# mjq11302010044/TPGSR

Measured on AMD Instinct MI355X. Metric: training img/s (16x64->32x128, bs=48/GPU), TPGSR-TSRN full train step, higher is better.
Workload: dtype bf16x2; 1 GPU; C3: TPGSR-TSRN = TSRN_TL (STN+mask) + CRNN teacher/student text prior, stu_iter 1, full train step (teacher fwd, student fwd+bwd, distill loss, prior dropout, SR fwd+bwd, ImageLoss(gradient), clip 0.25, Adam); tpg=crnn, batch_per_gpu=48, global_batch=48, parallelism=dp1, launch=recorded plans, plain launches: main + weight-gradient + teacher streams

## Files before the change

### tpgsr_amd/csrc/conv_route.cpp

```cpp
#include "conv_route.h"
#include <stdint.h>
#include <stdlib.h>
#include <initializer_list>

static inline int cdiv(long long a, long long b) { return (int)((a + b - 1) / b); }

static bool env_off(const char* name) { const char* e = getenv(name); return e && e[0] == '0'; }
static bool env_on(const char* name) { const char* e = getenv(name); return e && e[0] == '1'; }
static long long env_ll(const char* name, long long dflt) { const char* e = getenv(name); return e ? atoll(e) : dflt; }

static ConvKnobs knobs_from_env() {
  ConvKnobs k;
  k.wstat = !env_off("TPGSR_CONV_WSTAT");
  const long long target = env_ll("TPGSR_WGRAD_TARGET", 0);
  k.wgrad_target = target > 0 ? target : 1024;
  k.halo3 = !env_off("TPGSR_XBF_HALO3");
  k.halo3_min_supertiles = env_ll("TPGSR_XBF_HALO3_MIN", 192);
  k.halo = !env_off("TPGSR_XBF_HALO");
  k.halo_min_taps = env_on("TPGSR_XBF_HALO_MINTAPS") ? 1 : 2;
  k.colmajor_min_bytes = 3ll << 20;
  k.panel = !env_off("TPGSR_XBF_PANEL");
  k.panel_min_m = env_ll("TPGSR_XBF_PANEL_MIN_M", 32768);
  k.panel_k192 = env_on("TPGSR_XBF_PANEL_K192");
  k.splitk = !env_off("TPGSR_XBF_SPLITK");
  k.splitk_target = (int)env_ll("TPGSR_XBF_SPLITK_TARGET", 640);
  k.splitk_min_chunks = (int)env_ll("TPGSR_XBF_SPLITK_MIN_CHUNKS", 6);
  k.splitk_max_tiles = (int)env_ll("TPGSR_XBF_SPLITK_MAX_TILES", 256);
  k.splitk_min_k = (int)env_ll("TPGSR_XBF_SPLITK_MIN_K", 24);
  k.splitk_over_halo = !env_off("TPGSR_XBF_SPLITK_OVER_HALO");
  k.wgrad3 = !env_off("TPGSR_XBF_WGRAD3");
  k.wgrad_halo = !env_off("TPGSR_XBF_WGRAD_HALO");
  k.wgrad_halo_minwork = env_ll("TPGSR_XBF_WGRAD_HALO_MINWORK", 16384);
  return k;
}
ConvKnobs g_conv_knobs = knobs_from_env();

extern "C" void tpgsr_halo3_set_enabled(int on) { g_conv_knobs.halo3 = on ? 1 : 0; }
extern "C" void tpgsr_halo_set_min_taps(int v) { g_conv_knobs.halo_min_taps = v < 1 ? 1 : v; }
extern "C" void tpgsr_halo_set_colmajor_min_bytes(long long v) { g_conv_knobs.colmajor_min_bytes = v; }
extern "C" void tpgsr_panel_set_enabled(int on) { g_conv_knobs.panel = on ? 1 : 0; }
extern "C" void tpgsr_panel_set_min_m(long long m) { g_conv_knobs.panel_min_m = m < 64 ? 64 : m; }
extern "C" void tpgsr_panel_set_k192(int on) { g_conv_knobs.panel_k192 = on ? 1 : 0; }
extern "C" void tpgsr_splitk_set_enabled(int on) { g_conv_knobs.splitk = on ? 1 : 0; }
extern "C" void tpgsr_wgrad3_set_enabled(int on) { g_conv_knobs.wgrad3 = on ? 1 : 0; }

int loader_bits(const tpgsr_conv_args* a) {
  return (a->in_scale ? 1 : 0) | (a->in_act ? 2 : 0) | (a->in2 ? 4 : 0) | (a->in_ps ? 8 : 0) | (a->in_b ? 16 : 0) | (a->in2_scale ? 32 : 0);
}

bool xbf_eligible(const tpgsr_conv_args* a) { return a->terms > 0 && a->wt_bf && (a->Cin & 3) == 0 && (a->wt_coff & 31) == 0; }

static int halo_capacity_of(const tpgsr_conv_args* a, int P) {
  const int Wp = a->OW + a->KW - 1, ohw = a->OH * a->OW;
  const int row_wraps = (a->OW % P == 0) ? 0 : (P - 1) / a->OW + 1;
  const int img_wraps = (ohw % P == 0) ? 0 : (P - 1) / ohw + 1;
  return P - 1 + row_wraps * (a->KW - 1) + img_wraps * (a->KH - 1) * Wp + (a->KH - 1) * Wp + a->KW;
}
int halo_capacity(const tpgsr_conv_args* a) { return halo_capacity_of(a, 64); }
int halo3_capacity(const tpgsr_conv_args* a) { return halo_capacity_of(a, 64 * kH3Tiles); }

void wgrad_plan(long long M, int K, int Cout, int* Z, int* MB) {
  const int kb = cdiv(K, kWgradWK), nb = cdiv(Cout, kConvBN);
  long long z = (g_conv_knobs.wgrad_target + (long long)kb * nb - 1) / ((long long)kb * nb);
  long long maxz = (M + 255) / 256;
  if (maxz > 256) maxz = 256;
  if (z > maxz) z = maxz;
  if (z < 1) z = 1;
  long long mb = (M + z - 1) / z;
  mb = (mb + kWgradWM - 1) / kWgradWM * kWgradWM;
  z = (M + mb - 1) / mb;
  *Z = (int)z;
  *MB = (int)mb;
}

int splitk_choice(long long M, int Cout, int kp) {
  const ConvKnobs& k = g_conv_knobs;
  const long long ntiles = cdiv(M, 64) * cdiv(Cout, 64);
  const int nchunks = kp / kConvKC;
  if (ntiles > k.splitk_max_tiles || nchunks < k.splitk_min_k) return 0;
  int S = (int)(k.splitk_target / ntiles);
  S = S < 2 ? 2 : S > 8 ? 8 : S;
  int cps = (nchunks + S - 1) / S;
  if (cps < k.splitk_min_chunks) cps = k.splitk_min_chunks;
  S = (nchunks + cps - 1) / cps;
  return S > 1 ? S : 0;
}

static constexpr unsigned long long ld_set(std::initializer_list<int> lds) {
  unsigned long long m = 0;
  for (int b : lds) m |= 1ull << b;
  return m;
}
static bool ld_in(int ld, unsigned long long set) { return (unsigned)ld < 64 && ((set >> ld) & 1); }
static constexpr unsigned long long kF32FwdLd = ld_set({0, 1, 2, 3, 4, 5, 7, 8, 17});
static constexpr unsigned long long kWgradTileLd = ld_set({0, 1, 2, 3, 4, 5, 7, 17});
static constexpr unsigned long long kXbfFwdLd = ld_set({0, 1, 2, 3, 4, 5, 7, 8, 17});
static constexpr unsigned long long kHaloLd = ld_set({0, 1, 2, 3, 4, 5, 7});
static constexpr unsigned long long kHalo3Ld = ld_set({0, 1, 2, 3, 4, 5, 7, 37});
static constexpr unsigned long long kPanelLd = ld_set({0, 1, 4, 17});
static constexpr unsigned long long kWgradBatchLd = ld_set({0, 1, 3});
bool wgrad_batch_has_ld(int ld) { return ld_in(ld, kWgradBatchLd); }

static int halo3_takes(const tpgsr_conv_args* a, long long M, int ld, int* lds_out) {
  const ConvKnobs& k = g_conv_knobs;
  const int T = a->terms, taps = a->KH * a->KW;
  if (!k.halo3 || T < 1 || T > 2 || taps < 3 || !(taps & 1) || a->wt_bf_cin != a->Cin || (a->Cin & 31) || a->stride_w > 1 || a->in_dil_w > 1 ||
      a->in_b || a->in_ps || !ld_in(ld, kHalo3Ld) || a->OW + a->KW - 1 < 8)
    return 0;
  if ((ld & 4) && a->out_ps) return 0;
  const int Lcap = halo3_capacity(a);
  const int lds = 2 * T * (32 * kH3Entries * 64) + 2 * kH3Tiles * 1024 + 8 * 4096;
  if (Lcap > 32 * kH3Entries || lds > 163840) return 0;
  const long long nst = (long long)cdiv(cdiv(M, 64), kH3Tiles) * cdiv(a->Cout, 64);
  if (nst < k.halo3_min_supertiles) return 0;
  *lds_out = lds;
  return Lcap;
}

static int halo_takes(const tpgsr_conv_args* a, int ld, int* lds_out) {
  const ConvKnobs& k = g_conv_knobs;
  const int taps = a->KH * a->KW;
  if (!k.halo || taps < k.halo_min_taps || (a->wt_bf_cin != a->Cin && !(taps == 1 && a->wt_bf_cin == 0)) || (a->Cin & 31) || a->stride_w > 1 ||
      a->in_dil_w > 1 || a->in_b || !(ld_in(ld, kHaloLd) || ld == 8) || a->OW + a->KW - 1 < 8)
    return 0;
  const int Lcap = halo_capacity(a);
  const long long lds = 2ll * a->terms * Lcap * 64 + 2048;
  if (Lcap > 32 * 7 || lds > 80 * 1024) return 0;
  *lds_out = (int)lds;
  return Lcap;
}

static int panel_takes(const tpgsr_conv_args* a, long long M, int ld, int* lds_out) {
  const ConvKnobs& k = g_conv_knobs;
  const int T = a->terms;
  if (!k.panel || a->KH * a->KW != 1 || a->wt_bf_cin != 0 || a->stride_w > 1 || a->in_dil_w > 1 || a->in_ps || a->pad_h || a->pad_w ||
      a->OH != a->H || a->OW != a->W || M < k.panel_min_m || T < 1 || T > 3)
    return 0;
  const int nb32 = (a->Cout + 31) >> 5, nq8 = a->kp >> 5;
  int nbw = 0;
  if ((nq8 == 2 || nq8 == 3) && nb32 <= 6) nbw = 3;
  else if (nq8 == 6 && nb32 <= 2 && k.panel_k192) nbw = 1;
  else return 0;
  if (!ld_in(ld, kPanelLd)) return 0;
  const int panel = T * 64 * (nq8 * 64 + 16), epilogue = (4 * 64 * nbw + 4 * 1024) * 4;
  *lds_out = panel > epilogue ? panel : epilogue;
  return nbw;
}

static bool wstat_takes(const tpgsr_conv_args* a, int ld) {
  return g_conv_knobs.wstat && ld == 0 && a->KH == 3 && a->KW == 3 && a->pad_h == 1 && a->pad_w == 1 && a->Cin == 64 && a->Cout == 64 &&
         a->W == 64 && a->OW == 64 && a->OH == a->H && a->in_dil_w <= 1 && a->stride_w <= 1 && !a->out_ps && a->out_act == TPGSR_ACT_NONE &&
         (a->wt_ld == 0 || a->wt_ld == 64) && a->wt_coff == 0 && (a->in_ld & 3) == 0 && (a->in_coff & 3) == 0 &&
         (((uintptr_t)a->in | (uintptr_t)a->wt) & 15) == 0;
}

static tpgsr_conv_route_t fwd_route(const tpgsr_conv_args* a, long long M, int ld, bool planning) {
  tpgsr_conv_route_t r = {};
  r.ld = ld;
  if (!xbf_eligible(a)) {
    const int wld = a->wt_ld > 0 ? a->wt_ld : a->Cout;
    const bool vecB = (wld & 3) == 0 && ((uintptr_t)a->wt & 15) == 0 && (a->wt_coff & 3) == 0;
    if (wstat_takes(a, ld)) {
      r.kernel = TPGSR_CONV_F32_WSTAT;
      r.lds_bytes = kWstatLdsBytes;
    } else if ((a->Cin & 3) != 0 || !vecB) {
      r.kernel = TPGSR_CONV_F32_SCALAR;
    } else {
      r.kernel = ld_in(ld, kF32FwdLd) ? TPGSR_CONV_F32_TILE : TPGSR_CONV_NONE;
    }
    return r;
  }
  if (!planning && a->sk_splits > 1) {
    r.kernel = ld_in(ld, kXbfFwdLd) ? TPGSR_CONV_XBF_SPLITK : TPGSR_CONV_NONE;
    r.splits = r.kernel ? a->sk_splits : 0;
    return r;
  }
  if ((r.lcap = halo3_takes(a, M, ld, &r.lds_bytes)) > 0) r.kernel = TPGSR_CONV_XBF_HALO3;
  else if ((r.lcap = halo_takes(a, ld, &r.lds_bytes)) > 0) r.kernel = TPGSR_CONV_XBF_HALO;
  else if ((r.nbw = panel_takes(a, M, ld, &r.lds_bytes)) > 0) r.kernel = TPGSR_CONV_XBF_PANEL;
  else r.kernel = ld_in(ld, kXbfFwdLd) ? TPGSR_CONV_XBF_TILE : TPGSR_CONV_NONE;
  int unused = 0;
  const ConvKnobs& k = g_conv_knobs;
  if (planning && k.splitk && a->terms <= 3 && a->bn_row_tiles <= 1 && !a->in2_scale && ld_in(ld, kXbfFwdLd) &&
      (r.kernel == TPGSR_CONV_XBF_TILE || (r.kernel == TPGSR_CONV_XBF_HALO && k.splitk_over_halo && !panel_takes(a, M, ld, &unused))))
    r.sk_plan = splitk_choice(M, a->Cout, a->kp);
  return r;
}

tpgsr_conv_route_t conv_fwd_route(const tpgsr_conv_args* a, long long M) { return fwd_route(a, M, loader_bits(a), false); }
tpgsr_conv_route_t conv_fwd_plan_route(const tpgsr_conv_args* a, long long M, int ld) { return fwd_route(a, M, ld, true); }

static bool wgrad_halo_shape_ok(const tpgsr_conv_args* a, int* Lcap_out) {
  const int taps = a->KH * a->KW;
  if ((long long)a->Cin * a->Cout < g_conv_knobs.wgrad_halo_minwork) return false;
  if (taps < 2 || taps > 12 || (a->Cin & 31) || a->stride_w > 1 || a->in_dil_w > 1 || a->in_ps || a->in_b || a->OW + a->KW - 1 < 8) return false;
  const int Lcap = halo_capacity(a);
  if (Lcap > 32 * 9) return false;
  *Lcap_out = Lcap;
  return true;
}

int wgrad_halo_plan(const tpgsr_conv_args* a, int cus, int* zsplits, long long* dy_bf_bytes) {
  int Lcap = 0;
  if (!g_conv_knobs.wgrad_halo || a->terms <= 0 || !wgrad_halo_shape_ok(a, &Lcap)) return 0;
  const long long M = (long long)a->N * a->OH * a->OW;
  const int tiles = cdiv(M, 64);
  const int groups = (a->Cin >> 5) * cdiv(a->Cout, 64);
  int Z = cus / groups;
  if (Z < 1) Z = 1;
  if (Z > tiles) Z = tiles;
  const int tpz = cdiv(tiles, Z);
  Z = cdiv(tiles, tpz);
  if (zsplits) *zsplits = Z;
  if (dy_bf_bytes) *dy_bf_bytes = 3ll * cdiv(M, 16) * cdiv(a->Cout, 32) * 1024;
  return 1;
}

tpgsr_wgrad_route_t conv_wgrad_route(const tpgsr_wgrad_args* w, long long M) {
  const tpgsr_conv_args* a = &w->c;
  const int K = a->KH * a->KW * a->Cin, T = a->terms;
  tpgsr_wgrad_route_t r = {};
  const int ld = r.ld = loader_bits(a);
  wgrad_plan(M, K, a->Cout, &r.Z, &r.MB);
  if (w->zsplits > 0) {
    r.Z = w->zsplits;
    r.MB = cdiv(cdiv(M, 64), r.Z) * 64;
  }
  r.vecY = (!w->dy_ps && (w->dy_ld & 3) == 0 && (w->dy_coff & 3) == 0 && w->dy_ld >= ((a->Cout + 3) & ~3) + w->dy_coff &&
            ((uintptr_t)w->dy & 15) == 0) ? 1 : 0;
  if (!(T > 0 && (a->Cin & 3) == 0 && (r.vecY || w->dy_ps))) {
    if ((a->Cin & 3) != 0 || (!r.vecY && !w->dy_ps)) r.kernel = TPGSR_WGRAD_F32_SCALAR;
    else r.kernel = ld_in(ld, kWgradTileLd) ? TPGSR_WGRAD_F32_TILE : TPGSR_WGRAD_NONE;
    return r;
  }
  int Lcap = 0;
  if (g_conv_knobs.wgrad_halo && w->zsplits > 0 && w->dy_bf && ld_in(ld, kHaloLd) && wgrad_halo_shape_ok(a, &Lcap) &&
      2ll * T * Lcap * 64 + 512 <= 150 * 1024) {
    r.kernel = TPGSR_WGRAD_XBF_HALO;
    r.lcap = Lcap;
    r.ne = Lcap <= 32 * 7 ? 7 : 9;
    r.lds_bytes = 2 * T * Lcap * 64 + 512;
  } else if (g_conv_knobs.wgrad3 && T <= 2 && K % (3 * kWgradWK) == 0 && (ld == 0 || ld == 1) && !w->dy_ps && a->in_dil_w <= 1 && a->stride_w <= 1 &&
             !a->in_ps && M * (long long)w->dy_ld * 4 <= 0x7fffffffll) {
    r.kernel = TPGSR_WGRAD_XBF_3K;
  } else {
    r.kernel = ld_in(ld, kWgradTileLd) ? TPGSR_WGRAD_XBF_TILE : TPGSR_WGRAD_NONE;
  }
  return r;
}

static long long pixels(const tpgsr_conv_args* a) { return (long long)a->N * a->OH * a->OW; }
static bool geometry_ok(const tpgsr_conv_args* a) { return a->N > 0 && a->OH > 0 && a->OW > 0 && a->Cin > 0 && a->Cout > 0 && a->KH > 0 && a->KW > 0; }

extern "C" int tpgsr_conv_route(const tpgsr_conv_args* a, tpgsr_conv_route_t* r) {
  if (!a || !r || !geometry_ok(a)) return -1;
  *r = conv_fwd_route(a, pixels(a));
  r->sk_plan = conv_fwd_plan_route(a, pixels(a), r->ld).sk_plan;
  return r->kernel;
}

extern "C" int tpgsr_conv_wgrad_route(const tpgsr_wgrad_args* w, tpgsr_wgrad_route_t* r) {
  if (!w || !r || !geometry_ok(&w->c)) return -1;
  *r = conv_wgrad_route(w, pixels(&w->c));
  return r->kernel;
}

extern "C" int tpgsr_halo_capacity(const tpgsr_conv_args* a) { return a ? halo_capacity(a) : -1; }

extern "C" int tpgsr_wgrad_splits(int M, int K, int Cout) {
  int Z, MB;
  wgrad_plan(M, K, Cout, &Z, &MB);
  return Z;
}

extern "C" int tpgsr_conv_splitk_plan(const tpgsr_conv_args* a, long long* bytes) {
  if (bytes) *bytes = 0;
  if (!a || !xbf_eligible(a)) return 0;
  const long long M = pixels(a);
  const int S = conv_fwd_plan_route(a, M, loader_bits(a) & ~32).sk_plan;
  if (S > 1 && bytes) *bytes = (long long)S * cdiv(M, 64) * cdiv(a->Cout, 64) * 256 * 16 * 4;
  return S;
}

extern "C" int tpgsr_conv_in2_scale_ok(const tpgsr_conv_args* a) {
  if (!a || !xbf_eligible(a) || !a->in2 || !a->in_scale || a->in_act || a->in_b) return 0;
  return conv_fwd_plan_route(a, pixels(a), 37).kernel == TPGSR_CONV_XBF_HALO3 ? 1 : 0;
}

extern "C" int tpgsr_conv_bn_row_tiles(const tpgsr_conv_args* a) {
  if (!a || !xbf_eligible(a)) return 1;
  return conv_fwd_plan_route(a, pixels(a), loader_bits(a) & ~32).kernel == TPGSR_CONV_XBF_HALO3 ? kH3Tiles : 1;
}
```

### tpgsr_amd/csrc/conv_xbf.hip

```cpp
#include "conv_loader.h"
#include <type_traits>
#include <utility>
#include <vector>
#include <mutex>

#include "conv_xbf_common.h"

__device__ __forceinline__ int xa_off(int row, int slot) { return row * 64 + ((slot ^ ((row >> 2) & 3)) << 4); }

template <int LD, int T, int WMB, int WNB, int SK = 0>
__global__ __launch_bounds__(256, (WMB * WNB == 1 ? 3 : WMB * WNB == 2 ? 2 : 1)) void conv_fwd_xbf_kernel(tpgsr_conv_args a, int M, int K) {
  constexpr int BMT = 64 * WMB, BNT = 64 * WNB;
  constexpr int A_PLANE = BMT * 64;
  constexpr int BUF = T * A_PLANE;
  constexpr int NQ = BMT / 32;
  constexpr bool TWO = (T == 3) && (WMB * WNB <= 2);
  constexpr int EPI = (4 * 64 * WNB + 4 * 1024) * 4;
  __shared__ __attribute__((aligned(16))) unsigned char xsm[2 * BUF > EPI ? 2 * BUF : EPI];
  const int tid = threadIdx.x;
  const int lane = tid & 63, wave = tid >> 6;
  const int wm = wave & 1, wn = wave >> 1;
  const int nbn = (a.Cout + BNT - 1) / BNT;
  const int ntile = SK ? (int)gridDim.x / a.sk_splits : (int)gridDim.x;
  const int skz = SK ? (int)blockIdx.x / ntile : 0;
// ... 626 lines not shown
}

template <int LD, int T>
__device__ __forceinline__ void conv_wgrad_xbf_body(const tpgsr_wgrad_args& w, const int M, const int K, const int MB, const unsigned bx,
                                                    const unsigned gx, unsigned char* Am, unsigned char* Ym) {
  const tpgsr_conv_args& a = w.c;
  const int tid = threadIdx.x;
  const int lane = tid & 63, wave = tid >> 6;
  const int wk = wave & 1, wn = wave >> 1;
  const int nkb = (K + WK - 1) / WK, nnb = (a.Cout + BN - 1) / BN;
  const int tile = xcd_remap(bx, gx);
  const int kblk = tile % nkb, nblk = (tile / nkb) % nnb, zblk = tile / (nkb * nnb);
  const int k0 = kblk * WK, n0 = nblk * BN;
  const int mbeg = zblk * MB;
  const int mend = min(M, mbeg + MB);

  const int aq = tid & 15;
  const int ap0 = tid >> 4;
  const KPos kp = kpos_init(a, (k0 >> 2) + aq);
  const int ac = kp.c;
  const int yc = (tid & 15) * 4;

  ARaw qa0, qa1;
  float4 ry0, ry1;
  float4 qs = make_float4(1.f, 1.f, 1.f, 1.f), qt = make_float4(0.f, 0.f, 0.f, 0.f);
  const int Wr_ = real_w(a);
  const size_t in_floats = a.in_ps ? (size_t)a.N * a.H * a.W * a.Cin : (size_t)a.N * a.H * Wr_ * a.in_ld;
  const __amdgpu_buffer_rsrc_t rs_in = make_rsrc(a.in, in_floats);
  const __amdgpu_buffer_rsrc_t rs_in2 = (LD & 16) ? make_rsrc(a.in_b, (size_t)a.N * Wr_ * a.in_b_ld)
                                                  : make_rsrc(a.in2 ? a.in2 : a.in, (size_t)a.N * a.H * Wr_ * a.in2_ld);
  const __amdgpu_buffer_rsrc_t rs_dy = make_rsrc(w.dy, w.dy_ps ? (size_t)M * a.Cout : (size_t)M * w.dy_ld);
  if ((LD & 1) && kp.kh < a.KH) {
    qs = *reinterpret_cast<const float4*>(a.in_scale + ac);
    qt = *reinterpret_cast<const float4*>(a.in_shift + ac);
  }
  const bool cok = n0 + yc < a.Cout;
  auto load_dy = [&](const PixelPos& p, int m) -> float4 {
    if (!w.dy_ps) return buf_load4(rs_dy, (p.valid && cok) ? ((unsigned)m * (unsigned)w.dy_ld + (unsigned)(w.dy_coff + n0 + yc)) * 4u : OOB_OFF);
    float4 v = make_float4(0.f, 0.f, 0.f, 0.f);
    if (!p.valid || !cok) return v;
    const int C4 = a.Cout >> 2, cs = (n0 + yc) >> 2;
    const size_t W2 = 2 * (size_t)a.OW;
    const float* b = w.dy + ((size_t)(p.n * 2 * a.OH + 2 * p.oh) * W2 + 2 * p.ow) * C4 + cs;
    v.x = b[0];
    v.y = b[C4];
    v.z = b[W2 * C4];
    v.w = b[W2 * C4 + C4];
    return v;
  };
  auto load_chunk = [&](int mc) {
    const int ma = mc + ap0, mb = mc + ap0 + 16;
    const PixelPos p0 = decode_pixel(a, ma, mend);
    const PixelPos p1 = decode_pixel(a, mb, mend);
    qa0 = load_a_raw<LD>(a, rs_in, rs_in2, p0, kp);
    qa1 = load_a_raw<LD>(a, rs_in, rs_in2, p1, kp);
    ry0 = load_dy(p0, ma);
    ry1 = load_dy(p1, mb);
  };
  float4 dbq = make_float4(0.f, 0.f, 0.f, 0.f);
  const bool want_db = (w.dbpart != nullptr) && kblk == 0;
  auto store_chunk = [&]() {
    const float4 v0 = finish_a<LD>(a, qa0, qs, qt);
    const float4 v1 = finish_a<LD>(a, qa1, qs, qt);
    uint2 h0[T], h1[T], y0[T], y1[T];
    split4<T>(v0, h0);
    split4<T>(v1, h1);
    split4<T>(ry0, y0);
    split4<T>(ry1, y1);
#pragma unroll
    for (int t = 0; t < T; ++t) {
      *reinterpret_cast<uint2*>(Am + t * XW_PLANE + ap0 * XW_ROW + aq * 8) = h0[t];
      *reinterpret_cast<uint2*>(Am + t * XW_PLANE + (ap0 + 16) * XW_ROW + aq * 8) = h1[t];
      *reinterpret_cast<uint2*>(Ym + t * XW_PLANE + ap0 * XW_ROW + aq * 8) = y0[t];
      *reinterpret_cast<uint2*>(Ym + t * XW_PLANE + (ap0 + 16) * XW_ROW + aq * 8) = y1[t];
    }
    if (want_db) {
      dbq.x += ry0.x + ry1.x;
      dbq.y += ry0.y + ry1.y;
      dbq.z += ry0.z + ry1.z;
      dbq.w += ry0.w + ry1.w;
    }
  };

  floatx16 acc;
#pragma unroll
  for (int i = 0; i < 16; ++i) acc[i] = 0.f;

  if (mbeg < mend) {
    load_chunk(mbeg);
    store_chunk();
  }
  __syncthreads();
  for (int mc = mbeg; mc < mend; mc += WM) {
    const bool more = mc + WM < mend;
    if (more) load_chunk(mc + WM);
#pragma unroll
    for (int mb = 0; mb < WM / 16; ++mb) {
      bf16x8 av[T], bv[T];
#pragma unroll
      for (int t = 0; t < T; ++t) {
        av[t] = frag_tr(Am + t * XW_PLANE, lane, wk * 32, mb);
        bv[t] = frag_tr(Ym + t * XW_PLANE, lane, wn * 32, mb);
      }
      acc = mfma_terms<T>(av, bv, acc);
    }
    __builtin_amdgcn_sched_barrier(0);
    __syncthreads();
    if (more) {
      store_chunk();
      __syncthreads();
    }
  }
  const int bcol = wn * 32 + (lane & 31);
  const int n = n0 + bcol;
  float* dst = w.part + (size_t)zblk * K * a.Cout;
  if (n < a.Cout) {
#pragma unroll
    for (int r = 0; r < 16; ++r) {
      int k = k0 + wk * 32 + (r & 3) + 8 * (r >> 2) + 4 * (lane >> 5);
      if (k < K) dst[(size_t)k * a.Cout + n] = acc[r];
    }
  }
  if (want_db) {
    float* red = reinterpret_cast<float*>(Am);
    *reinterpret_cast<float4*>(red + ap0 * 64 + yc) = dbq;
    __syncthreads();
    if (tid < BN && n0 + tid < a.Cout) {
      float sdb = 0.f;
#pragma unroll
      for (int r = 0; r < 16; ++r) sdb += red[r * 64 + tid];
      w.dbpart[(size_t)zblk * a.Cout + n0 + tid] = sdb;
    }
  }
}

template <int LD, int T>
__global__ __launch_bounds__(256) void conv_wgrad_xbf_kernel(tpgsr_wgrad_args w, int M, int K, int MB) {
  __shared__ __attribute__((aligned(16))) unsigned char Am[T * XW_PLANE];
  __shared__ __attribute__((aligned(16))) unsigned char Ym[T * XW_PLANE];
  conv_wgrad_xbf_body<LD, T>(w, M, K, MB, blockIdx.x, gridDim.x, Am, Ym);
}

template <int LD, int T>
__global__ __launch_bounds__(256) void conv_wgrad_xbf3_kernel(tpgsr_wgrad_args w, int M, int K, int MB) {
  __shared__ __attribute__((aligned(16))) unsigned char Am[3][T * XW_PLANE];
  __shared__ __attribute__((aligned(16))) unsigned char Ym[T * XW_PLANE];
  const tpgsr_conv_args& a = w.c;
  const int tid = threadIdx.x;
  const int lane = tid & 63, wave = tid >> 6;
  const int wk = wave & 1, wn = wave >> 1;
  const int nkb = K / (3 * WK), nnb = (a.Cout + BN - 1) / BN;
  const int tile = xcd_remap(blockIdx.x, gridDim.x);
  const int kblk = tile % nkb, nblk = (tile / nkb) % nnb, zblk = tile / (nkb * nnb);
  const int k0 = kblk * 3 * WK, n0 = nblk * BN;
  const int mbeg = zblk * MB;
  const int mend = min(M, mbeg + MB);
  const int aq = tid & 15, ap0 = tid >> 4, yc = (tid & 15) * 4;

  int dih[3], diw[3], coff[3];
  float4 qs[3], qt[3];
#pragma unroll
  for (int j = 0; j < 3; ++j) {
    const KPos kp = kpos_init(a, ((k0 + j * WK) >> 2) + aq);
    dih[j] = kp.kh - a.pad_h;
    diw[j] = kp.kw - a.pad_w;
    coff[j] = a.in_coff + kp.c;
    qs[j] = make_float4(1.f, 1.f, 1.f, 1.f);
    qt[j] = make_float4(0.f, 0.f, 0.f, 0.f);
    if (LD & 1) {
      qs[j] = *reinterpret_cast<const float4*>(a.in_scale + kp.c);
      qt[j] = *reinterpret_cast<const float4*>(a.in_shift + kp.c);
    }
  }
  const __amdgpu_buffer_rsrc_t rs_in = make_rsrc(a.in, (size_t)a.N * a.H * a.W * a.in_ld);
  const __amdgpu_buffer_rsrc_t rs_dy = make_rsrc(w.dy, (size_t)M * w.dy_ld);
  const bool cok = n0 + yc < a.Cout;

  int pm[2], pn[2], poh[2], pow_[2];
#pragma unroll
  for (int r = 0; r < 2; ++r) {
    const int m = mbeg + ap0 + 16 * r, ohw = a.OH * a.OW;
    pm[r] = m;
    pn[r] = m / ohw;
    const int rem = m - pn[r] * ohw;
    poh[r] = rem / a.OW;
    pow_[r] = rem - poh[r] * a.OW;
  }
  float4 qa[2][3], ry[2];
  bool qok[2][3];
  auto load_chunk = [&]() __attribute__((always_inline)) {
#pragma unroll
    for (int r = 0; r < 2; ++r) {
      const bool valid = pm[r] < mend;
#pragma unroll
      for (int j = 0; j < 3; ++j) {
        const int ih = poh[r] + dih[j], iw = pow_[r] + diw[j];
        const bool ok = valid && (unsigned)ih < (unsigned)a.H && (unsigned)iw < (unsigned)a.W;
        qok[r][j] = ok;
        qa[r][j] = buf_load4(rs_in, ok ? ((unsigned)((pn[r] * a.H + ih) * a.W + iw) * (unsigned)a.in_ld + (unsigned)coff[j]) * 4u : OOB_OFF);
      }
      ry[r] = buf_load4(rs_dy, (valid && cok) ? ((unsigned)pm[r] * (unsigned)w.dy_ld + (unsigned)(w.dy_coff + n0 + yc)) * 4u : OOB_OFF);
      pm[r] += WM;
      pow_[r] += WM;
      while (pow_[r] >= a.OW) {
        pow_[r] -= a.OW;
        if (++poh[r] == a.OH) {
          poh[r] = 0;
          ++pn[r];
        }
      }
    }
  };
  float4 dbq = make_float4(0.f, 0.f, 0.f, 0.f);
  const bool want_db = (w.dbpart != nullptr) && kblk == 0;
  auto store_chunk = [&]() __attribute__((always_inline)) {
#pragma unroll
    for (int r = 0; r < 2; ++r) {
      const int row = ap0 + 16 * r;
#pragma unroll
      for (int j = 0; j < 3; ++j) {
        float4 v = qa[r][j];
        if (LD & 1) {
          v.x = qok[r][j] ? v.x * qs[j].x + qt[j].x : 0.f;
          v.y = qok[r][j] ? v.y * qs[j].y + qt[j].y : 0.f;
          v.z = qok[r][j] ? v.z * qs[j].z + qt[j].z : 0.f;
          v.w = qok[r][j] ? v.w * qs[j].w + qt[j].w : 0.f;
        }
        uint2 h[T];
        split4<T>(v, h);
#pragma unroll
        for (int t = 0; t < T; ++t) *reinterpret_cast<uint2*>(Am[j] + t * XW_PLANE + row * XW_ROW + aq * 8) = h[t];
      }
      uint2 y[T];
      split4<T>(ry[r], y);
#pragma unroll
      for (int t = 0; t < T; ++t) *reinterpret_cast<uint2*>(Ym + t * XW_PLANE + row * XW_ROW + aq * 8) = y[t];
    }
    if (want_db) {
      dbq.x += ry[0].x + ry[1].x;
      dbq.y += ry[0].y + ry[1].y;
      dbq.z += ry[0].z + ry[1].z;
      dbq.w += ry[0].w + ry[1].w;
    }
  };

  floatx16 acc[3];
#pragma unroll
  for (int j = 0; j < 3; ++j)
#pragma unroll
    for (int i = 0; i < 16; ++i) acc[j][i] = 0.f;

  if (mbeg < mend) {
    load_chunk();
    store_chunk();
  }
  __syncthreads();
  for (int mc = mbeg; mc < mend; mc += WM) {
    const bool more = mc + WM < mend;
    if (more) load_chunk();
#pragma unroll
    for (int mb = 0; mb < WM / 16; ++mb) {
      bf16x8 bv[T];
#pragma unroll
      for (int t = 0; t < T; ++t) bv[t] = frag_tr(Ym + t * XW_PLANE, lane, wn * 32, mb);
#pragma unroll
      for (int j = 0; j < 3; ++j) {
        bf16x8 av[T];
#pragma unroll
        for (int t = 0; t < T; ++t) av[t] = frag_tr(Am[j] + t * XW_PLANE, lane, wk * 32, mb);
        acc[j] = mfma_terms<T>(av, bv, acc[j]);
      }
    }
    __builtin_amdgcn_sched_barrier(0);
    __syncthreads();
    if (more) {
      store_chunk();
      __syncthreads();
    }
  }
  const int n = n0 + wn * 32 + (lane & 31);
  float* dst = w.part + (size_t)zblk * K * a.Cout;
  if (n < a.Cout) {
#pragma unroll
    for (int j = 0; j < 3; ++j)
#pragma unroll
      for (int r = 0; r < 16; ++r) {
        const int k = k0 + j * WK + wk * 32 + (r & 3) + 8 * (r >> 2) + 4 * (lane >> 5);
        dst[(size_t)k * a.Cout + n] = acc[j][r];
      }
  }
  if (want_db) {
    float* red = reinterpret_cast<float*>(Am[0]);
    *reinterpret_cast<float4*>(red + ap0 * 64 + yc) = dbq;
    __syncthreads();
    if (tid < BN && n0 + tid < a.Cout) {
      float sdb = 0.f;
#pragma unroll
      for (int r = 0; r < 16; ++r) sdb += red[r * 64 + tid];
      w.dbpart[(size_t)zblk * a.Cout + n0 + tid] = sdb;
    }
  }
}

template <int LD, int T>
__global__ __launch_bounds__(256) void conv_wgrad_xbf_batch_kernel(const tpgsr_wgrad_batch_item* __restrict__ items, int n) {
  __shared__ __attribute__((aligned(16))) unsigned char Am[T * XW_PLANE];
  __shared__ __attribute__((aligned(16))) unsigned char Ym[T * XW_PLANE];
  __shared__ int s_d;
  if (threadIdx.x == 0) {
    int lo = 0, hi = n - 1;
    while (lo < hi) {
      int mid = (lo + hi + 1) >> 1;
      if (items[mid].blk0 <= (int)blockIdx.x) lo = mid; else hi = mid - 1;
    }
    s_d = lo;
  }
  __syncthreads();
  const tpgsr_wgrad_batch_item* it = items + s_d;
  const tpgsr_wgrad_args w = it->w;
  conv_wgrad_xbf_body<LD, T>(w, it->M, it->K, it->MB, blockIdx.x - (unsigned)it->blk0, (unsigned)it->nblk, Am, Ym);
}

extern "C" int tpgsr_conv_wgrad_batch_prepare(const tpgsr_wgrad_args* w, tpgsr_wgrad_batch_item* item) {
  TPGSR_CHECK_ARG(w && item && w->dy && w->part, "tpgsr_conv_wgrad_batch_prepare: null pointer");
  const tpgsr_conv_args* a = &w->c;
  const long long M = (long long)a->N * a->OH * a->OW;
  const int K = a->KH * a->KW * a->Cin;
  const tpgsr_wgrad_route_t r = conv_wgrad_route(w, M);
  if (!((r.kernel == TPGSR_WGRAD_XBF_TILE || r.kernel == TPGSR_WGRAD_XBF_3K) && a->terms <= 3 && a->KH * a->KW == 1 && r.vecY && M < (1ll << 31) &&
        M * w->dy_ld * 4 <= 0x7fffffffll && a->wt_bf_cin == 0 && !w->dy_bf && wgrad_batch_has_ld(r.ld))) {
    tpgsr_set_error("tpgsr_conv_wgrad_batch_prepare: not a tile-loop split-bf16 launch with a loader variant the batch kernel has");
    return TPGSR_ERR_ARG;
  }
  item->w = *w;
  item->M = (int)M;
  item->K = K;
  item->MB = r.MB;
  item->blk0 = 0;
  item->nblk = cdiv(K, WK) * cdiv(a->Cout, BN) * r.Z;
  return r.ld;
}

extern "C" int tpgsr_conv_wgrad_batch(const tpgsr_wgrad_batch_item* items_dev, int n, int total_blocks, int ld, int terms, void* stream) {
  TPGSR_CHECK_ARG(items_dev && n > 0 && total_blocks > 0 && terms >= 1 && terms <= 3, "tpgsr_conv_wgrad_batch: bad arguments");
  hipStream_t st = (hipStream_t)stream;
  dim3 grid(total_blocks);
#define XBF_WGB_CASE(B)                                                                                                 \
  case B:                                                                                                               \
    if (terms == 1) hipLaunchKernelGGL((conv_wgrad_xbf_batch_kernel<B, 1>), grid, dim3(256), 0, st, items_dev, n);      \
    else if (terms == 2) hipLaunchKernelGGL((conv_wgrad_xbf_batch_kernel<B, 2>), grid, dim3(256), 0, st, items_dev, n); \
    else hipLaunchKernelGGL((conv_wgrad_xbf_batch_kernel<B, 3>), grid, dim3(256), 0, st, items_dev, n);                 \
    break;
  switch (ld) {
    XBF_WGB_CASE(0) XBF_WGB_CASE(1) XBF_WGB_CASE(3)
    default: return unsupported_ld("tpgsr_conv_wgrad_batch", ld);
  }
#undef XBF_WGB_CASE
  TPGSR_LAUNCH_CHECK("tpgsr_conv_wgrad_batch");
}

int conv_wgrad_xbf_launch(const tpgsr_wgrad_args* w, long long M, int K, const tpgsr_wgrad_route_t& r, hipStream_t st) {
  const tpgsr_conv_args* a = &w->c;
  const int T = a->terms, ld = r.ld, Z = r.Z, MB = r.MB;
  if (r.kernel == TPGSR_WGRAD_XBF_3K) {
    dim3 grid3((K / (3 * WK)) * cdiv(a->Cout, BN) * Z);
    if (ld == 0) {
      if (T == 1) hipLaunchKernelGGL((conv_wgrad_xbf3_kernel<0, 1>), grid3, dim3(256), 0, st, *w, (int)M, K, MB);
      else hipLaunchKernelGGL((conv_wgrad_xbf3_kernel<0, 2>), grid3, dim3(256), 0, st, *w, (int)M, K, MB);
    } else {
      if (T == 1) hipLaunchKernelGGL((conv_wgrad_xbf3_kernel<1, 1>), grid3, dim3(256), 0, st, *w, (int)M, K, MB);
      else hipLaunchKernelGGL((conv_wgrad_xbf3_kernel<1, 2>), grid3, dim3(256), 0, st, *w, (int)M, K, MB);
    }
    TPGSR_LAUNCH_CHECK("tpgsr_conv_wgrad(bf16 MFMA, three k-blocks)");
  }
  dim3 grid(cdiv(K, WK) * cdiv(a->Cout, BN) * Z);
#define XBF_WG_CASE(B)                                                                                       \
  case B:                                                                                                    \
    if (T == 1) hipLaunchKernelGGL((conv_wgrad_xbf_kernel<B, 1>), grid, dim3(256), 0, st, *w, (int)M, K, MB); \
    else if (T == 2) hipLaunchKernelGGL((conv_wgrad_xbf_kernel<B, 2>), grid, dim3(256), 0, st, *w, (int)M, K, MB); \
    else hipLaunchKernelGGL((conv_wgrad_xbf_kernel<B, 3>), grid, dim3(256), 0, st, *w, (int)M, K, MB);        \
    break;
  switch (ld) {
    XBF_WG_CASE(0) XBF_WG_CASE(1) XBF_WG_CASE(2) XBF_WG_CASE(3) XBF_WG_CASE(4) XBF_WG_CASE(5) XBF_WG_CASE(7) XBF_WG_CASE(17)
    default: return unsupported_ld("tpgsr_conv_wgrad", ld);
  }
#undef XBF_WG_CASE
  TPGSR_LAUNCH_CHECK("tpgsr_conv_wgrad(bf16 MFMA)");
}

template <int T>
__global__ __launch_bounds__(256) void dy_split_kernel(const float* __restrict__ dy, int dy_ld, int dy_coff, int dy_ps, int M, int Cout,
                                                       int OH, int OW, unsigned short* __restrict__ out, int MB16, int NB32) {
  const int lane = threadIdx.x & 63;
  const long long b = (long long)blockIdx.x * 4 + (threadIdx.x >> 6);
  if (b >= (long long)MB16 * NB32) return;
  const int mb = (int)(b / NB32), nb = (int)(b - (long long)mb * NB32);
  const int n = nb * 32 + (lane & 31), p0 = mb * 16 + (lane >> 5) * 8;
  __bf16 h[8][T];
#pragma unroll
  for (int j = 0; j < 8; ++j) {
    const int m = p0 + j;
    float v = 0.f;
    if (m < M && n < Cout) {
      if (!dy_ps) {
        v = dy[(size_t)m * dy_ld + dy_coff + n];
      } else {
        const int ohw = OH * OW, nn = m / ohw, rem = m - nn * ohw, oh = rem / OW, ow = rem - oh * OW;
        v = dy[((size_t)(nn * 2 * OH + 2 * oh + ((n >> 1) & 1)) * (2 * OW) + 2 * ow + (n & 1)) * (Cout >> 2) + (n >> 2)];
      }
    }
    split_bf<T>(v, h[j]);
  }
  const size_t plane = (size_t)MB16 * NB32 * 512;
#pragma unroll
  for (int t = 0; t < T; ++t) {
    bf16x8 v;
#pragma unroll
    for (int j = 0; j < 8; ++j) v[j] = h[j][t];
    *reinterpret_cast<bf16x8*>(out + t * plane + ((size_t)b * 64 + lane) * 8) = v;
  }
}

struct FastDiv {
  unsigned mul, sh;
};
static FastDiv fastdiv_make(unsigned d) {
  FastDiv f;
  unsigned l = 0;
  while ((1ull << l) < d) ++l;
  f.sh = l;
  f.mul = (unsigned)((((1ull << l) - d) << 32) / d + 1);
  return f;
}
__device__ __forceinline__ int fastdiv(int n, const FastDiv f) {
  const unsigned t = __umulhi((unsigned)n, f.mul);
  return (int)((t + (unsigned)n) >> f.sh);
}
struct HaloDivs {
  FastDiv ohw, ow, hpwp, wp;
};

#ifdef TPGSR_LAB
__device__ int g_wgh_dbg = 0;
extern "C" int tpgsr_wgh_debug(int bits) {
  return hipMemcpyToSymbol(HIP_SYMBOL(g_wgh_dbg), &bits, sizeof(bits)) == hipSuccess ? 0 : TPGSR_ERR_LAUNCH;
}
#define WGH_DBG() __builtin_amdgcn_readfirstlane(g_wgh_dbg)
#else
#define WGH_DBG() 0
#endif

template <int LD, int T, int NE>
__global__ __launch_bounds__(768, 3) void conv_wgrad_halo_kernel(tpgsr_wgrad_args w, int M, int Lcap, int Z, HaloDivs dv) {
  extern __shared__ __attribute__((aligned(16))) unsigned char hsm[];
  const tpgsr_conv_args& a = w.c;
  const int dbg = WGH_DBG();
  const int PLANE = Lcap * 64, BUF = T * PLANE;
  int* etab = reinterpret_cast<int*>(hsm + 2 * BUF);
  const int tid = threadIdx.x;
  const int lane = tid & 63, wave = __builtin_amdgcn_readfirstlane(tid >> 6);
  const int nnb = (a.Cout + 63) >> 6, NC = a.Cin >> 5;
  const int blk = xcd_remap(blockIdx.x, gridDim.x);
  const int nbk = blk % nnb, cc = (blk / nnb) % NC, z = blk / (nnb * NC);
  const int n0 = nbk * 64;
  const int tiles = (M + 63) >> 6, tpz = (tiles + Z - 1) / Z;
  const int t_beg = z * tpz, t_end = min(tiles, t_beg + tpz);
  const int taps = a.KH * a.KW;
  const int Hp = a.OH + a.KH - 1, Wp = a.OW + a.KW - 1, ohw = a.OH * a.OW;
  const int K = taps * a.Cin;
  auto qbase = [&](int m) __attribute__((always_inline)) {
    const int n = fastdiv(m, dv.ohw), r = m - n * ohw, oh = fastdiv(r, dv.ow);
    return (n * Hp + oh) * Wp + (r - oh * a.OW);
  };

  if (wave >= 8) {
    const int pt = tid - 512, aq = pt & 7, er = pt >> 3;
    const __amdgpu_buffer_rsrc_t rs_in = make_rsrc(a.in, (size_t)a.N * a.H * a.W * a.in_ld);
    const __amdgpu_buffer_rsrc_t rs_in2 = make_rsrc(a.in2 ? a.in2 : a.in, (size_t)a.N * a.H * a.W * a.in2_ld);
    const int c = cc * 32 + aq * 4;
    float4 qs = make_float4(1.f, 1.f, 1.f, 1.f), qt = make_float4(0.f, 0.f, 0.f, 0.f);
    if (LD & 1) {
      qs = *reinterpret_cast<const float4*>(a.in_scale + c);
      qt = *reinterpret_cast<const float4*>(a.in_shift + c);
    }
    int hpix[NE];
    int q0 = 0;
    auto decode_tile = [&](const int t) __attribute__((always_inline)) {
      const int m0 = t * 64;
      q0 = qbase(m0);
      const int L = qbase(min(m0 + 63, M - 1)) - q0 + (a.KH - 1) * Wp + a.KW;
      const int q = q0 + er * NE;
      int n = fastdiv(q, dv.hpwp);
      const int rem = q - n * (Hp * Wp);
      int r = fastdiv(rem, dv.wp), sx = rem - r * Wp;
      int rowbase = (n * a.H + r - a.pad_h) * a.W - a.pad_w;
      const int img_step = (Hp - a.H) * a.W;
#pragma unroll
      for (int i = 0; i < NE; ++i) {
        const int ih = r - a.pad_h, iw = sx - a.pad_w;
        const bool in = n < a.N && (unsigned)ih < (unsigned)a.H && (unsigned)iw < (unsigned)a.W;
        hpix[i] = er * NE + i < L ? (in ? rowbase + sx : -1) : -2;
        const bool c1 = ++sx >= Wp;
        sx = c1 ? 0 : sx;
        r += c1 ? 1 : 0;
        rowbase += c1 ? a.W : 0;
        const bool c2 = r >= Hp;
        r = c2 ? 0 : r;
        n += c2 ? 1 : 0;
        rowbase -= c2 ? img_step : 0;
      }
    };
    constexpr bool DB = !(LD & 4);
    ARaw hr[DB ? 2 : 1][NE];
    int tab[2] = {0, 0};
    auto load_item = [&](auto set_tag, const int t) __attribute__((always_inline)) {
      constexpr int S = decltype(set_tag)::value;
#pragma unroll
      for (int i = 0; i < NE; ++i) {
        const bool ok = hpix[i] >= 0;
        hr[S][i].ok = ok;
        hr[S][i].raw = hpix[i] > -2;
        hr[S][i].v = buf_load4(rs_in, ok ? ((unsigned)hpix[i] * (unsigned)a.in_ld + (unsigned)(a.in_coff + c)) * 4u : OOB_OFF);
        if (LD & 4) hr[S][i].v2 = buf_load4(rs_in2, ok ? ((unsigned)hpix[i] * (unsigned)a.in2_ld + (unsigned)c) * 4u : OOB_OFF);
      }
      tab[S] = pt < 64 ? qbase(min(t * 64 + pt, M - 1)) - q0 : 0;
    };
    auto store_item = [&](auto set_tag, const int j) __attribute__((always_inline)) {
      constexpr int S = decltype(set_tag)::value;
      unsigned char* buf = hsm + (j & 1) * BUF;
#pragma unroll
      for (int i = 0; i < NE; ++i) {
        const bool part = hr[S][i].raw;
        hr[S][i].raw = false;
        const float4 v = finish_a<LD>(a, hr[S][i], qs, qt);
        uint2 h[T];
        split4<T>(v, h);
        const int e = er * NE + i;
        const int off = e * 64 + (((aq >> 1) ^ ((e >> 2) & 3)) << 4) + (aq & 1) * 8;
        if (part) {
#pragma unroll
          for (int t = 0; t < T; ++t) *reinterpret_cast<uint2*>(buf + t * PLANE + off) = h[t];
        }
      }
      if (pt < 64) etab[(j & 1) * 64 + pt] = tab[S];
    };
    using P0 = std::integral_constant<int, 0>;
    using PN = std::integral_constant<int, DB ? 1 : 0>;
    int t = t_beg, j = 0;
    if (t < t_end) {
      decode_tile(t);
      if (DB) load_item(P0{}, t);
      auto item = [&](auto cur_tag, auto nxt_tag) __attribute__((always_inline)) -> bool {
        const bool more = t + 1 < t_end;
        if (!DB) load_item(cur_tag, t);
        if (more) decode_tile(t + 1);
        if (DB && more && !(dbg & 2)) load_item(nxt_tag, t + 1);
        if (!(dbg & 4)) store_item(cur_tag, j);
        __syncthreads();
        ++j;
        ++t;
        return more;
      };
      while (true) {
        if (!item(P0{}, PN{})) break;
        if (!item(PN{}, P0{})) break;
      }
    }
    return;
  }

  const int wn = wave & 1, tg = wave >> 1;
  const int TPG = (taps + 3) >> 2;
  const int tap0 = tg * TPG, ntap = max(0, min(taps, tap0 + TPG) - tap0);
  int tapoff[3];
#pragma unroll
  for (int i = 0; i < 3; ++i) {
    const int tp = min(tap0 + i, taps - 1);
    tapoff[i] = (tp / a.KW) * Wp + tp % a.KW;
  }
  const int NB32 = (a.Cout + 31) >> 5, MB16 = (M + 15) >> 4;
  const int nb32 = (n0 >> 5) + wn;
  const bool ncol = nb32 < NB32;
  const size_t plane_y = (size_t)MB16 * NB32 * 1024;
  const __amdgpu_buffer_rsrc_t rs_y = make_rsrc(reinterpret_cast<const float*>(w.dy_bf), (size_t)T * MB16 * NB32 * 256);
  const bool want_db = w.dbpart != nullptr && cc == 0 && tg == 0;
  const int G = lane >> 4, q = lane & 15;
  const int prow = (G >> 1) * 8 + (q >> 2);
  const int c0 = (G & 1) * 16 + (q & 3) * 4;
  auto a_off = [&](const int e) __attribute__((always_inline)) { return e * 64 + (((c0 >> 3) ^ ((e >> 2) & 3)) << 4) + (c0 & 4) * 2; };

  floatx16 acc[3], accdb;
#pragma unroll
  for (int r = 0; r < 16; ++r) acc[0][r] = acc[1][r] = acc[2][r] = accdb[r] = 0.f;
  u32x4 by[2][T];
  bf16x8 av[2][T];
  auto fetch_y = [&](auto set_tag, const int mb16) __attribute__((always_inline)) {
    constexpr int S = decltype(set_tag)::value;
#pragma unroll
    for (int t = 0; t < T; ++t) {
      const size_t off = t * plane_y + ((size_t)mb16 * NB32 + nb32) * 1024 + lane * 16;
      by[S][t] = __builtin_amdgcn_raw_buffer_load_b128(rs_y, (ncol && mb16 < MB16) ? (int)off : (int)OOB_OFF, 0, 0);
    }
  };
  auto fetch_a = [&](auto set_tag, const unsigned char* buf, const int e_lo, const int e_hi) __attribute__((always_inline)) {
    constexpr int S = decltype(set_tag)::value;
    const int o_lo = a_off(e_lo), o_hi = a_off(e_hi);
#pragma unroll
    for (int t = 0; t < T; ++t) {
      s16x4 lo = __builtin_amdgcn_ds_read_tr16_b64_v4i16((lds_s16x4_ptr)(buf + t * PLANE + o_lo));
      s16x4 hi = __builtin_amdgcn_ds_read_tr16_b64_v4i16((lds_s16x4_ptr)(buf + t * PLANE + o_hi));
      typedef short s16x8 __attribute__((ext_vector_type(8)));
      s16x8 v = __builtin_shufflevector(lo, hi, 0, 1, 2, 3, 4, 5, 6, 7);
      av[S][t] = __builtin_bit_cast(bf16x8, v);
    }
  };
  using I0 = std::integral_constant<int, 0>;
  using I1 = std::integral_constant<int, 1>;
  bf16x8 ones;
#pragma unroll
  for (int i = 0; i < 8; ++i) ones[i] = (__bf16)1.0f;

  int j = 0;
  if (t_beg < t_end) fetch_y(I0{}, t_beg * 4);
  for (int t = t_beg; t < t_end; ++t, ++j) {
    __syncthreads();
    const unsigned char* buf = hsm + (j & 1) * BUF;
    int e8[4][2];
#pragma unroll
    for (int s = 0; s < 4; ++s) {
      e8[s][0] = etab[(j & 1) * 64 + s * 16 + prow];
      e8[s][1] = etab[(j & 1) * 64 + s * 16 + prow + 4];
    }
    auto step = [&](auto ys_tag, const int s, const int mb16) __attribute__((always_inline)) {
      constexpr int YS = decltype(ys_tag)::value;
      fetch_y(std::integral_constant<int, YS ^ 1>{}, mb16 + 1);
      if (ntap > 0) fetch_a(I0{}, buf, e8[s][0] + tapoff[0], e8[s][1] + tapoff[0]);
      __builtin_amdgcn_sched_barrier(0);
      bf16x8 bv[T];
#pragma unroll
      for (int t2 = 0; t2 < T; ++t2) bv[t2] = __builtin_bit_cast(bf16x8, by[YS][t2]);
      if (want_db) {
#pragma unroll
        for (int t2 = T - 1; t2 >= 0; --t2) accdb = __builtin_amdgcn_mfma_f32_32x32x16_bf16(ones, bv[t2], accdb, 0, 0, 0);
      }
      if (ntap > 0) {
        if (ntap > 1) fetch_a(I1{}, buf, e8[s][0] + tapoff[1], e8[s][1] + tapoff[1]);
        __builtin_amdgcn_sched_barrier(0);
        acc[0] = mfma_terms<T>(av[0], bv, acc[0]);
        __builtin_amdgcn_sched_barrier(0);
        if (ntap > 1) {
          if (ntap > 2) fetch_a(I0{}, buf, e8[s][0] + tapoff[2], e8[s][1] + tapoff[2]);
          __builtin_amdgcn_sched_barrier(0);
          acc[1] = mfma_terms<T>(av[1], bv, acc[1]);
          __builtin_amdgcn_sched_barrier(0);
          if (ntap > 2) {
            acc[2] = mfma_terms<T>(av[0], bv, acc[2]);
            __builtin_amdgcn_sched_barrier(0);
          }
        }
      }
    };
    if (!(dbg & 1)) {
      step(I0{}, 0, t * 4 + 0);
      step(I1{}, 1, t * 4 + 1);
      step(I0{}, 2, t * 4 + 2);
      step(I1{}, 3, t * 4 + 3);
    }
  }
// ... 173 lines not shown
```

Measured before the change: 8814 img/s.

## Add shared-row wgrad kernel for 3x3 convs reusing one A row across kw taps

```diff
diff --git a/tpgsr_amd/csrc/conv_route.cpp b/tpgsr_amd/csrc/conv_route.cpp
--- a/tpgsr_amd/csrc/conv_route.cpp
+++ b/tpgsr_amd/csrc/conv_route.cpp
@@ -28,7 +28,7 @@
   k.splitk_max_tiles = (int)env_ll("TPGSR_XBF_SPLITK_MAX_TILES", 256);
   k.splitk_min_k = (int)env_ll("TPGSR_XBF_SPLITK_MIN_K", 24);
   k.splitk_over_halo = !env_off("TPGSR_XBF_SPLITK_OVER_HALO");
-  k.wgrad3 = !env_off("TPGSR_XBF_WGRAD3");
+  k.wgrad3 = env_off("TPGSR_XBF_WGRAD3") ? 0 : env_ll("TPGSR_XBF_WGRAD3", 1) == 2 ? 2 : 1;
   k.wgrad_halo = !env_off("TPGSR_XBF_WGRAD_HALO");
   k.wgrad_halo_minwork = env_ll("TPGSR_XBF_WGRAD_HALO_MINWORK", 16384);
   return k;
@@ -42,7 +42,7 @@
 extern "C" void tpgsr_panel_set_min_m(long long m) { g_conv_knobs.panel_min_m = m < 64 ? 64 : m; }
 extern "C" void tpgsr_panel_set_k192(int on) { g_conv_knobs.panel_k192 = on ? 1 : 0; }
 extern "C" void tpgsr_splitk_set_enabled(int on) { g_conv_knobs.splitk = on ? 1 : 0; }
-extern "C" void tpgsr_wgrad3_set_enabled(int on) { g_conv_knobs.wgrad3 = on ? 1 : 0; }
+extern "C" void tpgsr_wgrad3_set_enabled(int on) { g_conv_knobs.wgrad3 = on == 2 ? 2 : on ? 1 : 0; }
 
 int loader_bits(const tpgsr_conv_args* a) {
   return (a->in_scale ? 1 : 0) | (a->in_act ? 2 : 0) | (a->in2 ? 4 : 0) | (a->in_ps ? 8 : 0) | (a->in_b ? 16 : 0) | (a->in2_scale ? 32 : 0);
diff --git a/tpgsr_amd/csrc/conv_xbf.hip b/tpgsr_amd/csrc/conv_xbf.hip
--- a/tpgsr_amd/csrc/conv_xbf.hip
+++ b/tpgsr_amd/csrc/conv_xbf.hip
@@ -952,6 +952,170 @@
   }
 }
 
+constexpr int kWgrad3Ring = 1;
+#define XW_AROWS 34
+#define XW_APLANE (XW_AROWS * XW_ROW)
+template <int LD, int T, int RD>
+__global__ __launch_bounds__(256, 2) void conv_wgrad_xbf3r_kernel(tpgsr_wgrad_args w, int M, int K, int MB) {
+  __shared__ __attribute__((aligned(16))) unsigned char Am[2][T * XW_APLANE];
+  __shared__ __attribute__((aligned(16))) unsigned char Ym[2][T * XW_PLANE];
+  const tpgsr_conv_args& a = w.c;
+  const int tid = threadIdx.x;
+  const int lane = tid & 63, wave = tid >> 6;
+  const int wk = wave & 1, wn = wave >> 1;
+  const int nkb = K / (3 * WK), nnb = (a.Cout + BN - 1) / BN;
+  const int tile = xcd_remap(blockIdx.x, gridDim.x);
+  const int kblk = tile % nkb, nblk = (tile / nkb) % nnb, zblk = tile / (nkb * nnb);
+  const int k0 = kblk * 3 * WK, n0 = nblk * BN;
+  const int mbeg = zblk * MB;
+  const int mend = min(M, mbeg + MB);
+  const int nc = mbeg < mend ? (mend - mbeg) / WM : 0;
+  const int aq = tid & 15, ap0 = tid >> 4, yc = (tid & 15) * 4;
+  const int dih = kblk - a.pad_h;
+
+  float4 qs = make_float4(1.f, 1.f, 1.f, 1.f), qt = make_float4(0.f, 0.f, 0.f, 0.f);
+  if (LD & 1) {
+    qs = *reinterpret_cast<const float4*>(a.in_scale + aq * 4);
+    qt = *reinterpret_cast<const float4*>(a.in_shift + aq * 4);
+  }
+  const __amdgpu_buffer_rsrc_t rs_in = make_rsrc(a.in, (size_t)a.N * a.H * a.W * a.in_ld);
+  const __amdgpu_buffer_rsrc_t rs_dy = make_rsrc(w.dy, (size_t)M * w.dy_ld);
+  const bool cok = n0 + yc < a.Cout;
+  const bool edge = tid < 32, left = tid < 16;
+  const int ebit = left ? 1 : edge ? 2 : 0;
+  const unsigned toff = ((unsigned)(ap0 * a.in_ld + a.in_coff + aq * 4)) * 4u, toff16 = toff + 64u * (unsigned)a.in_ld;
+  const unsigned eoff = ((unsigned)((left ? -1 : WM) * a.in_ld + a.in_coff + aq * 4)) * 4u;
+  const unsigned yoff = ((unsigned)(ap0 * w.dy_ld + w.dy_coff + n0 + yc)) * 4u, yoff16 = yoff + 64u * (unsigned)w.dy_ld;
+  const int arow = (ap0 + 1) * XW_ROW + aq * 8, erow = (left ? 0 : XW_AROWS - 1) * XW_ROW + aq * 8, yrow = ap0 * XW_ROW + aq * 8;
+
+  int lm = mbeg, ln, loh, low0;
+  {
+    const int ohw = a.OH * a.OW;
+    ln = mbeg / ohw;
+    const int rem = mbeg - ln * ohw;
+    loh = rem / a.OW;
+    low0 = rem - loh * a.OW;
+  }
+  float4 qa[RD][3], ry[RD][2];
+  bool rok[RD], eok[RD];
+  auto load_chunk = [&](int s) __attribute__((always_inline)) {
+    const int ih = loh + dih;
+    const bool valid = lm < mend;
+    rok[s] = valid & ((unsigned)ih < (unsigned)a.H);
+    eok[s] = rok[s] & ((ebit & ((low0 > 0 ? 1 : 0) | (low0 + WM < a.W ? 2 : 0))) != 0);
+    const unsigned base = (unsigned)((ln * a.H + ih) * a.W + low0) * (unsigned)a.in_ld * 4u;
+    qa[s][0] = buf_load4(rs_in, rok[s] ? base + toff : OOB_OFF);
+    qa[s][1] = buf_load4(rs_in, rok[s] ? base + toff16 : OOB_OFF);
+    qa[s][2] = buf_load4(rs_in, eok[s] ? base + eoff : OOB_OFF);
+    const unsigned yb = (unsigned)lm * (unsigned)w.dy_ld * 4u;
+    const bool yok = valid & cok;
+    ry[s][0] = buf_load4(rs_dy, yok ? yb + yoff : OOB_OFF);
+    ry[s][1] = buf_load4(rs_dy, yok ? yb + yoff16 : OOB_OFF);
+    lm += WM;
+    low0 += WM;
+    const bool wrap_w = low0 == a.OW;
+    low0 = wrap_w ? 0 : low0;
+    loh += wrap_w ? 1 : 0;
+    const bool wrap_h = loh == a.OH;
+    loh = wrap_h ? 0 : loh;
+    ln += wrap_h ? 1 : 0;
+  };
+  float4 dbq = make_float4(0.f, 0.f, 0.f, 0.f);
+  const bool want_db = (w.dbpart != nullptr) && kblk == 0;
+  auto stage_a = [&](float4 v, bool ok, unsigned char* dst) __attribute__((always_inline)) {
+    if (LD & 1) {
+      v.x = ok ? v.x * qs.x + qt.x : 0.f;
+      v.y = ok ? v.y * qs.y + qt.y : 0.f;
+      v.z = ok ? v.z * qs.z + qt.z : 0.f;
+      v.w = ok ? v.w * qs.w + qt.w : 0.f;
+    }
+    uint2 h[T];
+    split4<T>(v, h);
+#pragma unroll
+    for (int t = 0; t < T; ++t) *reinterpret_cast<uint2*>(dst + t * XW_APLANE) = h[t];
+  };
+  auto store_chunk = [&](int s, int b) __attribute__((always_inline)) {
+#pragma unroll
+    for (int r = 0; r < 2; ++r) {
+      stage_a(qa[s][r], rok[s], Am[b] + arow + 16 * r * XW_ROW);
+      uint2 y[T];
+      split4<T>(ry[s][r], y);
+#pragma unroll
+      for (int t = 0; t < T; ++t) *reinterpret_cast<uint2*>(Ym[b] + t * XW_PLANE + yrow + 16 * r * XW_ROW) = y[t];
+    }
+    if (edge) stage_a(qa[s][2], eok[s], Am[b] + erow);
+    if (want_db) {
+      dbq.x += ry[s][0].x + ry[s][1].x;
+      dbq.y += ry[s][0].y + ry[s][1].y;
+      dbq.z += ry[s][0].z + ry[s][1].z;
+      dbq.w += ry[s][0].w + ry[s][1].w;
+    }
+  };
+
+  floatx16 acc[3];
+#pragma unroll
+  for (int j = 0; j < 3; ++j)
+#pragma unroll
+    for (int i = 0; i < 16; ++i) acc[j][i] = 0.f;
+
+#pragma unroll
+  for (int s = 0; s < RD; ++s) load_chunk(s);
+  store_chunk(0, 0);
+  load_chunk(0);
+  __syncthreads();
+  auto step = [&](int u) __attribute__((always_inline)) {
+    const int b = u & 1, s = (u + 1) % RD;
+#pragma unroll
+    for (int mb = 0; mb < WM / 16; ++mb) {
+      bf16x8 bv[T];
+#pragma unroll
+      for (int t = 0; t < T; ++t) bv[t] = frag_tr(Ym[b] + t * XW_PLANE, lane, wn * 32, mb);
+#pragma unroll
+      for (int j = 0; j < 3; ++j) {
+        bf16x8 av[T];
+#pragma unroll
+        for (int t = 0; t < T; ++t) av[t] = frag_tr(Am[b] + t * XW_APLANE + j * XW_ROW, lane, wk * 32, mb);
+        acc[j] = mfma_terms<T>(av, bv, acc[j]);
+      }
+    }
+    store_chunk(s, b ^ 1);
+    load_chunk(s);
+    __syncthreads();
+  };
+  constexpr int U = (RD & 1) ? 2 * RD : RD;
+  int c = 0;
+  for (; c + U <= nc; c += U) {
+#pragma unroll
+    for (int u = 0; u < U; ++u) step(u);
+  }
+#pragma unroll
+  for (int u = 0; u < U - 1; ++u)
+    if (c + u < nc) step(u);
+
+  const int n = n0 + wn * 32 + (lane & 31);
+  float* dst = w.part + (size_t)zblk * K * a.Cout;
+  if (n < a.Cout) {
+#pragma unroll
+    for (int j = 0; j < 3; ++j)
+#pragma unroll
+      for (int r = 0; r < 16; ++r) {
+        const int k = k0 + j * WK + wk * 32 + (r & 3) + 8 * (r >> 2) + 4 * (lane >> 5);
+        dst[(size_t)k * a.Cout + n] = acc[j][r];
+      }
+  }
+  if (want_db) {
+    float* red = reinterpret_cast<float*>(Am[0]);
+    *reinterpret_cast<float4*>(red + ap0 * 64 + yc) = dbq;
+    __syncthreads();
+    if (tid < BN && n0 + tid < a.Cout) {
+      float sdb = 0.f;
+#pragma unroll
+      for (int r = 0; r < 16; ++r) sdb += red[r * 64 + tid];
+      w.dbpart[(size_t)zblk * a.Cout + n0 + tid] = sdb;
+    }
+  }
+}
+
 template <int LD, int T>
 __global__ __launch_bounds__(256) void conv_wgrad_xbf_batch_kernel(const tpgsr_wgrad_batch_item* __restrict__ items, int n) {
   __shared__ __attribute__((aligned(16))) unsigned char Am[T * XW_PLANE];
@@ -1014,6 +1178,16 @@
   const int T = a->terms, ld = r.ld, Z = r.Z, MB = r.MB;
   if (r.kernel == TPGSR_WGRAD_XBF_3K) {
     dim3 grid3((K / (3 * WK)) * cdiv(a->Cout, BN) * Z);
+    if (g_conv_knobs.wgrad3 == 1 && a->Cin == 64 && a->KW == 3 && a->pad_w == 1 && a->W == a->OW && a->OW % WM == 0 && MB % WM == 0) {
+      if (ld == 0) {
+        if (T == 1) hipLaunchKernelGGL((conv_wgrad_xbf3r_kernel<0, 1, kWgrad3Ring>), grid3, dim3(256), 0, st, *w, (int)M, K, MB);
+        else hipLaunchKernelGGL((conv_wgrad_xbf3r_kernel<0, 2, kWgrad3Ring>), grid3, dim3(256), 0, st, *w, (int)M, K, MB);
+      } else {
+        if (T == 1) hipLaunchKernelGGL((conv_wgrad_xbf3r_kernel<1, 1, kWgrad3Ring>), grid3, dim3(256), 0, st, *w, (int)M, K, MB);
+        else hipLaunchKernelGGL((conv_wgrad_xbf3r_kernel<1, 2, kWgrad3Ring>), grid3, dim3(256), 0, st, *w, (int)M, K, MB);
+      }
+      TPGSR_LAUNCH_CHECK("tpgsr_conv_wgrad(bf16 MFMA, three k-blocks, shared rows)");
+    }
     if (ld == 0) {
       if (T == 1) hipLaunchKernelGGL((conv_wgrad_xbf3_kernel<0, 1>), grid3, dim3(256), 0, st, *w, (int)M, K, MB);
       else hipLaunchKernelGGL((conv_wgrad_xbf3_kernel<0, 2>), grid3, dim3(256), 0, st, *w, (int)M, K, MB);
```

Result: no change. 8839 img/s (median of 6 runs) (+0.3%).
